# nevi-me/rust-dataframe

Hardware: AMD Instinct MI355X
Metric: rows/sec filter+sum over 1e9 f64 Arrow rows; %HBM bw at 1/2/4/8 GPU (higher is better)
Workload: dtype f64

## Files before the change

rust_dataframe_amd/csrc/rdf_capi.cpp:

```cpp
#include <hip/hip_runtime.h>

#include <algorithm>
#include <cmath>
#include <cstdarg>
#include <cstdio>
#include <chrono>
#include <functional>
#include <cstring>
#include <map>
#include <memory>
#include <mutex>
#include <condition_variable>
#include <string>
#include <thread>
#include <vector>
#include <sys/syscall.h>
#include <unistd.h>

#include "rdf_device.h"
#include "rdf_stage_copy.h"
#include "rdf_stream_plan.h"
#include "rdf_join_place.h"
#include "rdf_program_plan.h"
#include "rdf_groupby_multi_plan.h"
// ... 30 lines not shown
    std::vector<void*> overflow;
};

struct Ctx {
    bool        ready = false;
    int         device = 0;
    hipStream_t own_stream = nullptr;
    hipStream_t stream = nullptr;
    hipStream_t copy_stream = nullptr;
    bool copy_pending = false;
    Arena       arena;
    char*       pinned = nullptr;
    size_t      pinned_cap = 0;
    std::string err;
    std::string last_kernel;
    bool   opt_spec = true;
    bool   opt_fast_filter = true;
    bool   opt_vec_bitmap = false;
    int    opt_filter_block = 1;
    int    opt_interp_lean = 1;
    int    opt_filter_owned = 1;
    int    opt_filter_ends = 1;
    int    opt_filter_short = 1;
    int    opt_filter_block_rows = 8192;
    int    opt_filter_fused = 1;
    int    opt_gbm_route = 0;
    int64_t opt_gbm_slots = 0;
    int    opt_gb_debug = 0;
    bool   sort_used_local = false;
    int64_t utf8_sort_rounds = 0;
// ... 43 lines not shown
    char* tab_pin = nullptr; size_t tab_pin_cap = 0, tab_pin_used = 0;
    bool   agg_comm_entered = false;
    ::rdf_comm* agg_comm = nullptr;
    ~Ctx();
};

thread_local Ctx g_ctx;

Ctx::~Ctx() {
    if (!ready || (long)syscall(SYS_gettid) == (long)getpid()) return;
    (void)hipSetDevice(device);
    if (stream) (void)hipStreamSynchronize(stream);
    for (void* p : arena.overflow) (void)hipFree(p);
    if (arena.base) (void)hipFree(arena.base);
    if (pinned) (void)hipHostFree(pinned);
    for (auto& kv : pool_free) (void)hipFree(kv.second);
    for (int b = 0; b < 2; ++b) { if (sbuf_dev[b]) (void)hipFree(sbuf_dev[b]); if (sbuf_pin[b]) (void)hipHostFree(sbuf_pin[b]); if (sbuf_ev[b]) (void)hipEventDestroy(sbuf_ev[b]); }
    if (tab_pin) (void)hipHostFree(tab_pin);
    if (d2h_stream) (void)hipStreamSynchronize(d2h_stream);
    for (int b = 0; b < 2; ++b) { if (dbuf_dev[b]) (void)hipFree(dbuf_dev[b]); if (dbuf_pin[b]) (void)hipHostFree(dbuf_pin[b]); if (dbuf_ev[b]) (void)hipEventDestroy(dbuf_ev[b]); }
    if (d2h_stream) (void)hipStreamDestroy(d2h_stream);
    for (auto& ev : events) { (void)hipEventDestroy(ev.first); (void)hipEventDestroy(ev.second); }
    if (copy_stream) { (void)hipStreamSynchronize(copy_stream); (void)hipStreamDestroy(copy_stream); }
    if (own_stream) (void)hipStreamDestroy(own_stream);
    ready = false;
}

rdf_status fail(rdf_status st, const char* fmt, ...) {
    char buf[512];
    va_list ap;
// ... 19 lines not shown
rdf_status ensure_ready() {
    Ctx& c = g_ctx;
    if (c.ready) return RDF_OK;
    int n = 0;
    hipError_t e = hipGetDeviceCount(&n);
    if (e != hipSuccess || n <= 0)
        return fail(RDF_DEVICE_ERROR, "no HIP device visible (%s); librdf_mi355x has no CPU fallback",
                    e != hipSuccess ? hipGetErrorString(e) : "device count 0");
    HIP_TRY(hipGetDevice(&c.device));
    hipDeviceProp_t prop;
    HIP_TRY(hipGetDeviceProperties(&prop, c.device));
    if (strncmp(prop.gcnArchName, "gfx950", 6) != 0)
        return fail(RDF_DEVICE_ERROR, "device %d is %s; this library carries gfx950 (MI355X) code only", c.device, prop.gcnArchName);
    HIP_TRY(hipStreamCreateWithFlags(&c.own_stream, hipStreamNonBlocking));
    c.stream = c.own_stream;
    if (const char* e = getenv("RDF_SPEC_BLOCKS_PER_CU")) { const int v = atoi(e); if (v >= 0 && v <= 8) c.opt_spec_blocks = v; }
    if (const char* e = getenv("RDF_SPEC_TILE_ROT")) c.opt_spec_tile_rot = atoi(e);
    if (const char* e = getenv("RDF_SPEC_XCD_SWZ")) c.opt_spec_xcd_swz = atoi(e);
    if (const char* e = getenv("RDF_SPEC_GRID_ADJ")) c.opt_spec_grid_adj = atoi(e);
    if (const char* e = getenv("RDF_STREAM_TABLE_KERNEL")) c.opt_stream_table_kernel = atoi(e) != 0;
    if (const char* e = getenv("RDF_GSPEC_BLOCKS_PER_CU")) { const int v = atoi(e); if (v >= 0 && v <= 8) c.opt_gspec_blocks = v; }
    c.ready = true;
    return RDF_OK;
}

void arena_begin() {
    Arena& a = g_ctx.arena;
    for (void* p : a.overflow) (void)hipFree(p);
    a.overflow.clear();
    if (a.wanted > a.cap) {
// ... 138 lines not shown
        for (auto& it : items) if (!it.small) { it.off = off; off += (it.bytes + 16 + 255) & ~(size_t)255; }
        total = off;
        void* p = nullptr;
        RDF_TRY(arena_alloc(total ? total : 256, &p));
        dev = (char*)p;
        return RDF_OK;
    }
    char* ptr(int idx) const { return dev + items[(size_t)idx].off; }

    rdf_status upload(size_t pinned_off, size_t* pinned_used) {
        Ctx& c = g_ctx;
        if (small_bytes) {
            char* pin = c.pinned + pinned_off;
            packed_copy(items, pin, true, small_bytes);
            HIP_TRY(hipMemcpyAsync(dev, pin, small_bytes, hipMemcpyHostToDevice, c.stream));
        }
        *pinned_used = small_bytes;
        for (auto& it : items)
            if (!it.small && it.bytes) HIP_TRY(hipMemcpyAsync(dev + it.off, it.src, it.bytes, hipMemcpyHostToDevice, c.stream));
        return RDF_OK;
    }
    rdf_status download(size_t pinned_off) {
        Ctx& c = g_ctx;
        if (small_bytes) HIP_TRY(hipMemcpyAsync(c.pinned + pinned_off, dev, small_bytes, hipMemcpyDeviceToHost, c.stream));
        for (auto& it : items)
            if (!it.small && it.bytes) HIP_TRY(hipMemcpyAsync((void*)it.src, dev + it.off, it.bytes, hipMemcpyDeviceToHost, c.stream));
        HIP_TRY(hipStreamSynchronize(c.stream));
        if (small_bytes) {
            packed_copy(items, c.pinned + pinned_off, false, small_bytes);
        }
        return RDF_OK;
    }
};

struct InPlan {
    int values_item = -1, validity_item = -1;
    int64_t dev_offset = 0;
};

struct DbgTimer {
    bool on;
    std::chrono::steady_clock::time_point t0;
    DbgTimer() : on(getenv("RDF_DEBUG") != nullptr), t0(std::chrono::steady_clock::now()) {}
    void mark(const char* what) {
        if (!on) return;
        const auto t1 = std::chrono::steady_clock::now();
        fprintf(stderr, "[rdf] %-28s %8.3f ms\n", what, std::chrono::duration<double, std::milli>(t1 - t0).count());
        t0 = t1;
    }
};

struct InputStager {
    Region region;
    std::vector<InPlan> plans;
    std::vector<const rdf_array*> arrays;
    std::vector<DevChunkCol> dev;
    bool host = false;

    void add(const rdf_array* a) {
        arrays.push_back(a);
        if (a->mem != RDF_MEM_HOST && !host) return;
        if (plans.size() + 1 < arrays.size()) plans.resize(arrays.size() - 1);
// ... 56 lines not shown
        return RDF_OK;
    }
    template <typename T> T* at(size_t off) { return (T*)(base + off); }
    template <typename T> T* dev_at(size_t off) const { return (T*)(dev + off); }
    rdf_status alloc() {
        void* p = nullptr;
        RDF_TRY(arena_alloc(size ? size : 16, &p));
        dev = (char*)p;
        return RDF_OK;
    }
    rdf_status upload(size_t pinned_off) {
        Ctx& c = g_ctx;
        if (size == 0) return RDF_OK;
        if (base != c.pinned + pinned_off) return fail(RDF_COMPUTE_ERROR, "internal: table builder not bound to its staging offset");
        HIP_TRY(hipMemcpyAsync(dev, base, size, hipMemcpyHostToDevice, c.stream));
        return RDF_OK;
    }
};

rdf_status check_mem(const rdf_array* arrs, int64_t n, int32_t* mem_io) {
    for (int64_t i = 0; i < n; ++i) {
        if (arrs[i].mem != RDF_MEM_HOST && arrs[i].mem != RDF_MEM_DEVICE) return fail(RDF_INVALID_ARGUMENT, "bad mem tag %d", arrs[i].mem);
        if (*mem_io < 0) *mem_io = arrs[i].mem;
        else if (*mem_io != arrs[i].mem) return fail(RDF_INVALID_ARGUMENT, "all arrays of one call must share one memory space");
        if (arrs[i].length < 0 || arrs[i].offset < 0) return fail(RDF_INVALID_ARGUMENT, "negative length/offset");
        if (arrs[i].length > 0 && arrs[i].values == nullptr) return fail(RDF_INVALID_ARGUMENT, "null values pointer");
    }
    return RDF_OK;
}
rdf_status check_out_mem(const rdf_out* outs, int64_t n, int32_t mem) {
// ... 120 lines not shown
    hipError_t e = hipGetDeviceCount(&n);
    *count = e == hipSuccess ? n : 0;
    if (e != hipSuccess) return fail(RDF_DEVICE_ERROR, "hipGetDeviceCount: %s", hipGetErrorString(e));
    return RDF_OK;
}

rdf_status rdf_set_device(int32_t device) {
    Ctx& c = g_ctx;
    if (c.ready && c.device == device) return RDF_OK;
    if (c.ready) {
        (void)hipStreamSynchronize(c.stream);
        for (void* p : c.arena.overflow) (void)hipFree(p);
        c.arena.overflow.clear();
        if (c.arena.base) (void)hipFree(c.arena.base);
        c.arena = Arena();
        for (auto& ev : c.events) { (void)hipEventDestroy(ev.first); (void)hipEventDestroy(ev.second); }
        c.events.clear();
        c.events_used = 0;
        if (c.own_stream) (void)hipStreamDestroy(c.own_stream);
        c.own_stream = c.stream = nullptr;
        c.ready = false;
    }
    HIP_TRY(hipSetDevice(device));
    return ensure_ready();
}

rdf_status rdf_set_stream(void* hip_stream) {
    RDF_TRY(ensure_ready());
    g_ctx.stream = hip_stream ? (hipStream_t)hip_stream : g_ctx.own_stream;
    return RDF_OK;
// ... 1903 lines not shown
```

rust_dataframe_amd/csrc/rdf_capi_program.inc:

```

namespace {


bool op_is_arith(int op) { return op >= RDF_OP_ADD && op <= RDF_OP_DIV; }
bool op_is_fbinary(int op) { return op >= RDF_OP_ATAN2 && op <= RDF_OP_LOG; }
bool op_is_unary_math(int op) { return (op >= RDF_OP_ABS && op <= RDF_OP_TANH) || (op >= RDF_OP_COT && op <= RDF_OP_CSC); }
bool op_is_cmp(int op) { return op >= RDF_OP_GT && op <= RDF_OP_LE; }
bool op_is_hour(int op) { return op >= RDF_OP_HOUR_S && op <= RDF_OP_HOUR_DAY; }
bool op_is_binary(int op) { return op_is_arith(op) || op_is_fbinary(op) || op_is_cmp(op) || op == RDF_OP_AND || op == RDF_OP_OR; }
bool op_is_heavy(int op) {
    if (op_is_fbinary(op)) return true;
    if (!op_is_unary_math(op)) return false;
    switch (op) {
        case RDF_OP_ABS: case RDF_OP_CEIL: case RDF_OP_FLOOR: case RDF_OP_ROUND: case RDF_OP_SQRT:
        case RDF_OP_DEGREES: case RDF_OP_RADIANS: return false;
        default: return true;
    }
}

struct Compiler {
    const rdf_expr_node* nodes;
    int nnodes;
    const int* col_dtype;
    int ncols;
// ... 486 lines not shown
                    else if (op == RDF_OP_DIV) h = sw ? LH_F_RDIV : LH_F_DIV;
                } else if (in.dtype == RDF_I64 || in.dtype == RDF_U64) {
                    if (op == RDF_OP_ADD) h = LH_I_ADD;
                    else if (op == RDF_OP_MUL) h = LH_I_MUL;
                    else if (op == RDF_OP_SUB) h = sw ? LH_I_RSUB : LH_I_SUB;
                }
            } break;
            default: break;
        }
        if (h == LH_NONE) return false;
        lean.code[i].swapped = (uint8_t)((in.swapped & 1) | (h << 1));
    }
    return true;
}

rdf_status launch_agg_pair(const EvalArgs* ea, const FilterAggF64Args* fa, int cmp, int feat, int grid, int nvalues,
                           const int* cls, AggPartial* partials, AggPartial* result, const char* spec_sig = nullptr,
                           const SpecArgs* sa = nullptr) {
    Ctx& c = g_ctx;
    KernelTimer kt;
    if (sa) {
        const bool jit = jit_find(spec_sig) != nullptr;
        c.last_kernel = std::string("spec_kernel<") + spec_sig + ">" + (jit ? " [compiled at run time]" : "");
        const hipError_t le = launch_spec(spec_sig, *sa, grid, c.stream);
        if (le != hipSuccess && jit) { (void)hipGetLastError(); return kRetryInterpreted; }
        if (le != hipSuccess) return fail(RDF_DEVICE_ERROR, "launch_spec: %s", hipGetErrorString(le));
    }
    else if (fa) { c.last_kernel = "filter_agg_f64_kernel"; HIP_TRY(launch_filter_agg_f64(*fa, cmp, grid, c.stream)); }
    else {
        EvalArgs lean;
        if (c.opt_interp_lean && feat == 0 && lean_assign(*ea, lean)) { c.last_kernel = "eval_kernel<AGG, lean>"; HIP_TRY(launch_eval_lean(lean, SINK_AGG, grid, c.stream, c.opt_interp_lean == 2)); }
        else { c.last_kernel = "eval_kernel<AGG>"; HIP_TRY(launch_eval(*ea, SINK_AGG, feat, grid, c.stream)); }
    }
    kt.stop();
    AggFinalArgs f;
    memset(&f, 0, sizeof f);
    f.partials = partials;
    f.result = result;
    f.nblocks = grid;
    f.nvalues = nvalues;
    for (int k = 0; k < nvalues; ++k) f.value_cls[k] = cls[k];
    HIP_TRY(launch_agg_final(f, c.stream));
    return RDF_OK;
}

void fill_agg_result(rdf_agg_result* r, int dt, const AggPartial& p) {
    memset(r, 0, sizeof *r);
    r->dtype = dt;
    r->count = p.cnt;
    r->is_some = p.cnt > 0;
    if (is_float(dt)) {
        double s, a, b;
        memcpy(&s, &p.sum, 8); memcpy(&a, &p.mn, 8); memcpy(&b, &p.mx, 8);
        r->sum_f64 = dt == RDF_F32 ? (double)(float)s : s;
        if (p.cnt > 0) { r->min_f64 = a; r->max_f64 = b; }
    } else {
        r->sum_i64 = (int64_t)h_normalize_int(dt, p.sum);
        if (p.cnt > 0) { r->min_i64 = (int64_t)p.mn; r->max_i64 = (int64_t)p.mx; }
// ... 26 lines not shown
    int cls[kMaxGroupValues] = {0, 0, 0, 0, 0, 0, 0, 0};
    size_t pin_off = 0;
    InputStager in;
    const std::vector<DevChunkCol>* in_dev = nullptr;
    Region outr;
    std::vector<DevOutChunk> dev_outs;
    std::vector<int> out_val_item, out_vld_item;
    std::vector<int64_t> tile_start;
    const rdf_frame::Tiles* eval_tiles = nullptr;
    int64_t ntiles = 0;
    int grid = 0;
    size_t n_nc = 0;
    int gwords = 0;
    void* scratch = nullptr;
    uint32_t* d_flags = nullptr;
    int64_t* d_nullc = nullptr;
    AggPartial* d_partials = nullptr;
    AggPartial* d_result = nullptr;
    EvalArgs ea;
    TableBuilder tb;
    bool use_spec = false;
    SpecPlan sp;
    int rt_ops[8] = {0, 0, 0, 0, 0, 0, 0, 0};
    SpecArgs sa;
    TableBuilder stb;

    ProgramRun(const ProgramSpec& p, const rdf_array* c, int nc, int64_t nch, rdf_out* o, rdf_agg_result* a, rdf_frame* f)
        : ps(p), cols(c), ncols(nc), nchunks(nch), outs(o), aggs(a), fc(f), grouped(p.sink == RDF_SINK_GROUP), cc(p.nodes, p.nnodes, col_dtype, nc) {}
};

rdf_status program_check(ProgramRun& r, const char* len_mismatch_msg) {
    const ProgramSpec& ps = r.ps;
    const rdf_array* cols = r.cols;
    const int ncols = r.ncols;
    const int64_t nchunks = r.nchunks;
    rdf_frame* fc = r.fc;
    if (nchunks < 0) return fail(RDF_INVALID_ARGUMENT, "negative chunk count");
    if (ncols < 0 || ncols > kMaxCols) return fail(RDF_INVALID_ARGUMENT, "a fused program reads at most %d columns", kMaxCols);
    if (ps.nvalues < 1 || ps.nvalues > (r.grouped ? kMaxGroupValues : kMaxValues)) return fail(RDF_INVALID_ARGUMENT, "nvalues out of range");
    if (r.grouped) {
        if (ps.ngroups < 1 || (int64_t)(ps.ngroups + 1) * ps.nvalues > RDF_MAX_GROUP_SLOTS)
            return fail(RDF_INVALID_ARGUMENT, "grouped aggregation: (ngroups + 1) * nvalues must be in [2, %d] (large key domains: rdf_groupby_sum)", RDF_MAX_GROUP_SLOTS);
        if (!ps.gout) return fail(RDF_INVALID_ARGUMENT, "null output pointer");
// ... 91 lines not shown

rdf_status program_flags_status(uint32_t flags, const ProgramSpec& ps) {
    if ((flags & 2u) && ps.sink == RDF_SINK_AGG && g_ctx.agg_comm) return fail(RDF_COMPUTE_ERROR, "pipeline_dist: another rank failed before the combine");
    if (flags & 1u) return fail(RDF_DIVIDE_BY_ZERO, "Divide by zero error");
    if ((flags & 2u) && ps.sink == RDF_SINK_GROUP) return fail(RDF_COMPUTE_ERROR, "group id outside [0, %d)", ps.ngroups);
    return RDF_OK;
}

rdf_status deliver_agg(ProgramRun& r, const AggPartial* d_result, const uint32_t* d_flags) {
    Ctx& ctx = g_ctx;
    const int nvalues = r.ps.nvalues;
    AggPartial hp[kMaxValues];
    uint32_t flags = 0;
    if (ctx.agg_comm) RDF_TRY(agg_dist_finish(*ctx.agg_comm, d_result, d_flags, nvalues, r.cls, hp, &flags));
    else {
        RDF_TRY(pinned_reserve(r.pin_off + 64 + sizeof(AggPartial) * kMaxValues));
        char* pin = ctx.pinned + r.pin_off;
        HIP_TRY(hipMemcpyAsync(pin, d_flags, 16, hipMemcpyDeviceToHost, ctx.stream));
        HIP_TRY(hipMemcpyAsync(pin + 64, d_result, sizeof(AggPartial) * (size_t)nvalues, hipMemcpyDeviceToHost, ctx.stream));
        HIP_TRY(hipStreamSynchronize(ctx.stream));
        r.dbg.mark("kernel + result");
        memcpy(&flags, pin, 4);
        memcpy(hp, pin + 64, sizeof(AggPartial) * (size_t)nvalues);
    }
    RDF_TRY(program_flags_status(flags, r.ps));
    for (int v = 0; v < nvalues; ++v) fill_agg_result(&r.aggs[v], r.value_dtype[v], hp[v]);
    return RDF_OK;
}

rdf_status program_empty(ProgramRun& r) {
    const ProgramSpec& ps = r.ps;
    if (r.frame_store) return RDF_OK;
    if (ps.sink == RDF_SINK_STORE) {
        for (int64_t i = 0; i < (int64_t)ps.nvalues * r.nchunks; ++i) { r.outs[i].length = 0; r.outs[i].null_count = 0; }
    } else if (r.grouped) {
        for (int v = 0; v < ps.nvalues; ++v)
            for (int g = 0; g <= ps.ngroups; ++g) {
                rdf_group_result& gr = ps.gout[(size_t)v * (size_t)(ps.ngroups + 1) + (size_t)g];
                memset(&gr, 0, sizeof gr);
                gr.dtype = r.value_dtype[v];
// ... 23 lines not shown
    }
    return RDF_OK;
}

rdf_status program_stage(ProgramRun& r) {
    const ProgramSpec& ps = r.ps;
    const int64_t nchunks = r.nchunks;
    const int ncols = r.ncols;
    rdf_frame* fc = r.fc;
    RDF_TRY(ensure_ready());
    Ctx& ctx = g_ctx;
    arena_begin();
    size_t pin_used = 0;
    if (!fc) {
        r.in.arrays.reserve((size_t)ncols * (size_t)nchunks);
        r.in.plans.reserve((size_t)ncols * (size_t)nchunks);
        for (int64_t i = 0; i < (int64_t)ncols * nchunks; ++i) r.in.add(&r.cols[i]);
        RDF_TRY(r.in.finish(r.pin_off, &pin_used));
        r.pin_off += (pin_used + 255) & ~(size_t)255;
    }
    r.in_dev = fc ? &fc->dev : &r.in.dev;
    r.dbg.mark("stage inputs");

    const std::vector<int64_t>& clen = *r.clen;
    std::vector<DevOutChunk>& dev_outs = r.dev_outs;
    if (r.frame_store) {
        if (nchunks == 1) { dev_outs.resize((size_t)ps.nvalues); for (int v = 0; v < ps.nvalues; ++v) dev_outs[(size_t)v] = ps.frame_out0[v]; }
    } else if (ps.sink == RDF_SINK_STORE) {
        dev_outs.resize((size_t)ps.nvalues * nchunks);
        if (r.mem == RDF_MEM_HOST) {
            r.out_val_item.assign(dev_outs.size(), -1);
// ... 6 lines not shown
                    const size_t vb = r.value_dtype[v] == RDF_BOOL ? (size_t)((n + 7) / 8) : (size_t)n * (size_t)dtype_size(r.value_dtype[v]);
                    r.out_val_item[i] = r.outr.add(r.outs[i].values, vb);
                    if (r.outs[i].validity) r.out_vld_item[i] = r.outr.add(r.outs[i].validity, (size_t)((n + 7) / 8));
                }
            RDF_TRY(r.outr.layout());
            for (size_t i = 0; i < dev_outs.size(); ++i) {
                dev_outs[i].values = r.out_val_item[i] >= 0 ? r.outr.ptr(r.out_val_item[i]) : nullptr;
                dev_outs[i].validity = r.out_vld_item[i] >= 0 ? (uint8_t*)r.outr.ptr(r.out_vld_item[i]) : nullptr;
            }
        } else {
            for (size_t i = 0; i < dev_outs.size(); ++i) dev_outs[i] = DevOutChunk{r.outs[i].values, r.outs[i].validity};
        }
    }

    if (fc) { RDF_TRY(frame_tiles(*fc, kEvalTile, &r.eval_tiles)); r.ntiles = r.eval_tiles->ntiles; }
    else {
        r.tile_start.assign((size_t)nchunks + 1, 0);
        r.ntiles = tile_prefix(clen.data(), nchunks, kEvalTile, r.tile_start.data());
    }
    r.grid = (int)(r.ntiles < (int64_t)eval_grid_limit() ? r.ntiles : (int64_t)eval_grid_limit());

    r.n_nc = ps.sink == RDF_SINK_STORE ? (size_t)ps.nvalues * (size_t)nchunks : 0;
    r.gwords = r.grouped ? group_words(ps.ngroups, ps.nvalues) : 0;
    const size_t scratch_bytes = 16 + r.n_nc * 8 + ((size_t)r.grid + 4) * (r.grouped ? (size_t)r.gwords * 8 : (size_t)ps.nvalues * sizeof(AggPartial));
    RDF_TRY(arena_alloc(scratch_bytes, &r.scratch));
    r.d_flags = (uint32_t*)r.scratch;
    r.d_nullc = (int64_t*)((char*)r.scratch + 16);
    r.d_partials = (AggPartial*)((char*)r.scratch + 16 + r.n_nc * 8);
    r.d_result = r.d_partials + (size_t)r.grid * (size_t)ps.nvalues;
    HIP_TRY(hipMemsetAsync(r.scratch, 0, 16 + r.n_nc * 8, ctx.stream));

    EvalArgs& ea = r.ea;
    memset(&ea, 0, sizeof ea);
    ea.nchunks = nchunks;
    ea.ntiles = r.ntiles;
    ea.ncols = ncols;
    ea.nvalues = ps.nvalues;
    ea.ncode = (int)r.cc.code.size();
    ea.ntmp = r.cc.tmp_max;
    ea.flags = r.d_flags;
    ea.out_null_counts = r.d_nullc;
    ea.partials = r.d_partials;
    for (int k = 0; k < ncols; ++k) ea.col_dtype[k] = r.col_dtype[k];
    for (int v = 0; v < ps.nvalues; ++v) ea.value_cls[v] = r.cls[v];
    memcpy(ea.code, r.cc.code.data(), r.cc.code.size() * sizeof(Instr));
// ... 102 lines not shown
    for (int k = 0; k < kSpecCols; ++k) {
        sa.alias[k] = -1;
        for (int j = 0; j < k && k < sp.ncols; ++j) if (sp.col_map[j] == sp.col_map[k]) { sa.alias[k] = j; break; }
    }
    sa.partials = r.d_partials;
    sa.flags = r.d_flags;
    sa.vec_bitmap = ctx.opt_vec_bitmap ? 1 : 0;
    sa.out_null_count = r.d_nullc;
    sa.nchunks = nchunks;
    std::vector<int64_t> sts;
    const rdf_frame::Tiles* spec_tiles = nullptr;
    if (fc) {
        RDF_TRY(frame_tiles(*fc, spec_rpb, &spec_tiles));
        sa.ntiles = spec_tiles->ntiles;
        sa.tile_inv = spec_tiles->tile_inv;
    } else {
        sts.assign((size_t)nchunks + 1, 0);
        sa.ntiles = tile_prefix(clen.data(), nchunks, spec_rpb, sts.data());
        sa.tile_inv = tile_reciprocal(nchunks, sts[(size_t)nchunks - 1]);
    }
    if (nchunks == 1) {
        for (int k = 0; k < sp.ncols; ++k) sa.cols[k] = in_dev[(size_t)sp.col_map[k]];
        sa.n = clen[0];
        if (ps.sink == RDF_SINK_STORE) sa.out = r.dev_outs[0];
    } else if (fc) {
        DevChunkCol* tab = nullptr;
        RDF_TRY(frame_col_tab(*fc, sp.col_map, sp.ncols, &tab));
        sa.cols_tab = tab;
        sa.chunk_tile_start = spec_tiles->d_start;
        sa.chunk_len = fc->d_clen;
// ... 33 lines not shown
    wi.nchunks = nchunks;
    wi.ncols = sp.ncols;
    wi.any_bitmap = false;
    for (int k = 0; k < sp.ncols; ++k) wi.any_bitmap |= fc ? fc->col_nullable[sp.col_map[k]] : in_dev[(size_t)((int64_t)sp.col_map[k] * nchunks)].validity != nullptr;
    wi.ntiles = sa.ntiles;
    wi.grid_limit = eval_grid_limit();
    wi.waves_per_block = kBlock / 64;
    wi.spec_blocks_per_cu = ctx.opt_spec_blocks;
    wi.spec_tile_rot = ctx.opt_spec_tile_rot;
    wi.spec_xcd_swz = ctx.opt_spec_xcd_swz;
    wi.spec_grid_adj = ctx.opt_spec_grid_adj;
    const WalkPlan wp = spec_walk_plan(wi);
    r.grid = wp.grid;
    sa.tile_rot = wp.tile_rot;
    sa.xcd_swz = wp.xcd_swz;
    r.d_result = r.d_partials + (size_t)r.grid * (size_t)ps.nvalues;
    return RDF_OK;
}

rdf_status run_group(ProgramRun& r) {
    const ProgramSpec& ps = r.ps;
    Ctx& ctx = g_ctx;
    EvalArgs& ea = r.ea;
    const int64_t nchunks = r.nchunks;
    const std::vector<DevChunkCol>& in_dev = *r.in_dev;
    const std::vector<int64_t>& clen = *r.clen;
    const int gwords = r.gwords;
    ea.ngroups = ps.ngroups;
    ea.group_replicas = group_replicas(gwords, r.cc.tmp_max);
    uint64_t* d_gpart = (uint64_t*)r.d_partials;
    uint64_t* d_gres = d_gpart + (size_t)r.grid * (size_t)gwords;
    ea.group_partials = d_gpart;
    SpecPlan gp;
    bool use_gspec = ctx.opt_spec && ps.ngroups <= 8 &&
                     build_gspec_plan(r.cc, ps.filter_root, ps.group_root, ps.ngroups, ps.nvalues, ps.value_roots, gp);
    for (int k = 0; k < gp.ncols && use_gspec; ++k) {
        const int w = dtype_size(r.col_dtype[gp.col_map[k]]);
        for (int64_t c = 0; c < nchunks; ++c) {
            const DevChunkCol& d = in_dev[(size_t)((int64_t)gp.col_map[k] * nchunks + c)];
            if (clen[(size_t)c] > 0 && ((uintptr_t)((const char*)d.values + d.offset * w) & (uintptr_t)(2 * w - 1)) != 0) { use_gspec = false; break; }
        }
    }
    if (use_gspec) {
        GSpecArgs ga;
        memset(&ga, 0, sizeof ga);
        ga.cols_tab = ea.cols; ga.chunk_tile_start = ea.chunk_tile_start; ga.chunk_len = ea.chunk_len;
        ga.nchunks = nchunks; ga.ntiles = r.ntiles; ga.n = clen[0];
        for (int k = 0; k < gp.ncols; ++k) { ga.col_map[k] = gp.col_map[k]; if (nchunks == 1) ga.cols[k] = in_dev[(size_t)gp.col_map[k]]; }
        for (int k = 0; k < gp.nimm; ++k) ga.imm[k] = gp.imm[k];
        ga.group_partials = d_gpart; ga.flags = r.d_flags;
        ga.ngroups = ps.ngroups; ga.nvalues = ps.nvalues; ga.vec_bitmap = ctx.opt_vec_bitmap ? 1 : 0;
        const WalkPlan wp = gspec_walk_plan(r.grid, eval_grid_limit(), ctx.opt_gspec_blocks, ctx.opt_spec_tile_rot, ctx.opt_spec_xcd_swz);
        r.grid = wp.grid;
        ga.xcd_swz = wp.xcd_swz;
        ga.tile_rot = wp.tile_rot;
        KernelTimer kt;
        ctx.last_kernel = "gspec_kernel<" + gp.sig + ">" + (jit_find(gp.sig.c_str()) ? " [compiled at run time]" : "");
        const hipError_t le = launch_gspec(gp.sig.c_str(), ga, r.grid, ctx.stream);
        if (le != hipSuccess && jit_find(gp.sig.c_str()) == nullptr && !gspec_available(gp.sig.c_str())) {
            (void)hipGetLastError();
            return kRetryInterpreted;
        }
        if (le != hipSuccess) return fail(RDF_DEVICE_ERROR, "launch_gspec: %s", hipGetErrorString(le));
        kt.stop();
    } else {
        KernelTimer kt;
        ctx.last_kernel = "eval_kernel<GROUP>";
        HIP_TRY(launch_eval(ea, SINK_GROUP, r.cc.feat(), r.grid, ctx.stream));
        kt.stop();
    }
    GroupFinalArgs gf;
    memset(&gf, 0, sizeof gf);
    gf.partials = d_gpart; gf.result = d_gres; gf.nblocks = r.grid; gf.words = gwords; gf.ngroups = ps.ngroups; gf.nvalues = ps.nvalues;
    for (int v = 0; v < ps.nvalues; ++v) gf.value_cls[v] = r.cls[v];
    HIP_TRY(launch_group_final(gf, ctx.stream));
    RDF_TRY(pinned_reserve(r.pin_off + 64 + (size_t)gwords * 8));
    char* pin = ctx.pinned + r.pin_off;
    HIP_TRY(hipMemcpyAsync(pin, r.d_flags, 16, hipMemcpyDeviceToHost, ctx.stream));
    HIP_TRY(hipMemcpyAsync(pin + 64, d_gres, (size_t)gwords * 8, hipMemcpyDeviceToHost, ctx.stream));
    HIP_TRY(hipStreamSynchronize(ctx.stream));
    uint32_t flags;
    memcpy(&flags, pin, 4);
    RDF_TRY(program_flags_status(flags, ps));
    const uint64_t* w = (const uint64_t*)(pin + 64);
    const int S = ps.ngroups + 1;
    for (int v = 0; v < ps.nvalues; ++v)
        for (int g = 0; g < S; ++g) {
            rdf_group_result& gr = ps.gout[(size_t)v * (size_t)S + (size_t)g];
            memset(&gr, 0, sizeof gr);
            gr.dtype = r.value_dtype[v];
            gr.count = (int64_t)(w[2 * ps.nvalues * S + g] - w[(ps.nvalues + v) * S + g]);
            gr.is_some = gr.count > 0;
            if (is_float(r.value_dtype[v])) memcpy(&gr.sum_f64, &w[v * S + g], 8);
            else gr.sum_i64 = (int64_t)w[v * S + g];
        }
    if (ps.grows) for (int g = 0; g < S; ++g) ps.grows[g] = (int64_t)w[2 * ps.nvalues * S + g];
    return RDF_OK;
}

// ... 16 lines not shown
    if (!(coln && r.col_dtype[coln->column] == RDF_F64 && sc->dtype != RDF_NULLTYPE && (is_numeric(sc->dtype) || sc->dtype == RDF_BOOL))) return false;
    const DevChunkCol& x = (*r.in_dev)[(size_t)coln->column];
    const DevChunkCol& y = (*r.in_dev)[(size_t)vr.column];
    const uintptr_t xa = (uintptr_t)((const double*)x.values + x.offset), ya = (uintptr_t)((const double*)y.values + y.offset);
    if (!((xa & 7) == 0 && (ya & 7) == 0 && (xa & 15) == (ya & 15))) return false;
    memset(&fa, 0, sizeof fa);
    fa.x = (const double*)x.values; fa.x_validity = x.validity; fa.x_offset = x.offset;
    fa.y = (const double*)y.values; fa.y_validity = y.validity; fa.y_offset = y.offset;
    fa.n = (*r.clen)[0];
    const uint64_t cu = r.cc.imm_for(*sc, RDF_F64);
    memcpy(&fa.c, &cu, 8);
    fa.partials = r.d_partials;
    return true;
}

rdf_status run_agg(ProgramRun& r) {
    const ProgramSpec& ps = r.ps;
    FilterAggF64Args fa;
    int cmp = 0;
    if (r.use_spec) {
        RDF_TRY(launch_agg_pair(nullptr, nullptr, 0, 0, r.grid, ps.nvalues, r.cls, r.d_partials, r.d_result, r.sp.sig.c_str(), &r.sa));
    } else if (fast_filter_match(r, fa, cmp)) {
        const int64_t per_block = (int64_t)kBlock * 4 * 2;
        const int64_t want = ((*r.clen)[0] + per_block - 1) / per_block;
        r.grid = (int)(want < (int64_t)eval_grid_limit() ? want : (int64_t)eval_grid_limit());
        if (r.grid < 1) r.grid = 1;
        r.d_result = r.d_partials + (size_t)r.grid * (size_t)ps.nvalues;
        RDF_TRY(launch_agg_pair(nullptr, &fa, cmp, 0, r.grid, 1, r.cls, r.d_partials, r.d_result));
    } else {
        RDF_TRY(launch_agg_pair(&r.ea, nullptr, 0, r.cc.feat(), r.grid, ps.nvalues, r.cls, r.d_partials, r.d_result));
    }
    return deliver_agg(r, r.d_result, r.d_flags);
}

rdf_status run_store(ProgramRun& r) {
    const ProgramSpec& ps = r.ps;
    Ctx& ctx = g_ctx;
    const int64_t nchunks = r.nchunks;
    const std::vector<int64_t>& clen = *r.clen;
    {
        KernelTimer kt;
        if (r.use_spec) {
            const bool jit = jit_find(r.sp.sig.c_str()) != nullptr;
            ctx.last_kernel = "spec_kernel<" + r.sp.sig + ">" + (jit ? " [compiled at run time]" : "");
            const hipError_t le = launch_spec(r.sp.sig.c_str(), r.sa, r.grid, ctx.stream);
            if (le != hipSuccess && jit) { (void)hipGetLastError(); return kRetryInterpreted; }
            if (le != hipSuccess) return fail(RDF_DEVICE_ERROR, "launch_spec: %s", hipGetErrorString(le));
        }
        else {
            int64_t longest = 0;
            for (int64_t i = 0; i < nchunks; ++i) longest = std::max(longest, clen[(size_t)i]);
            EvalArgs lean;
            if (ctx.opt_interp_lean && r.cc.feat() == 0 && longest < ((int64_t)1 << 32) && lean_assign(r.ea, lean, SINK_STORE)) {
                ctx.last_kernel = "eval_kernel<STORE, lean>";
                HIP_TRY(launch_eval_lean(lean, SINK_STORE, r.grid, ctx.stream, ctx.opt_interp_lean == 2));
            } else { ctx.last_kernel = "eval_kernel<STORE>"; HIP_TRY(launch_eval(r.ea, SINK_STORE, r.cc.feat(), r.grid, ctx.stream)); }
        }
        kt.stop();
    }
    const size_t head = r.frame_store ? 16 : 16 + r.n_nc * 8;
    RDF_TRY(pinned_reserve(r.pin_off + 64 + (r.frame_store ? 0 : r.n_nc * 8 + r.outr.small_bytes + 256)));
    char* pin = ctx.pinned + r.pin_off;
    HIP_TRY(hipMemcpyAsync(pin, r.scratch, head, hipMemcpyDeviceToHost, ctx.stream));
    if (!r.frame_store && r.mem == RDF_MEM_HOST) RDF_TRY(r.outr.download(r.pin_off + ((head + 255) & ~(size_t)255)));
    else HIP_TRY(hipStreamSynchronize(ctx.stream));
    uint32_t flags;
    memcpy(&flags, pin, 4);
    RDF_TRY(program_flags_status(flags, ps));
    if (r.frame_store) return RDF_OK;
    for (int v = 0; v < ps.nvalues; ++v)
        for (int64_t c = 0; c < nchunks; ++c) {
            rdf_out& o = r.outs[(int64_t)v * nchunks + c];
            o.length = clen[(size_t)c];
            memcpy(&o.null_count, pin + 16 + 8 * (size_t)((int64_t)v * nchunks + c), 8);
        }
    return RDF_OK;
}

// ... 87 lines not shown
```

rust_dataframe_amd/csrc/rdf_device.h:

```cpp
#pragma once
#include "rdf_sort_map.h"
#include <stdint.h>
#include <hip/hip_runtime.h>

#include <string>
#include "../../include/rdf_mi355x.h"

namespace rdfk {

constexpr int kBlock = 256;
constexpr int kVPT = 4;
constexpr int kEvalTile = kBlock * kVPT;
constexpr int kFilterTile = 4096;
constexpr int kMaxCode = 56;
constexpr int kMaxCols = 8;
constexpr int kMaxFrameCols = 64;
constexpr int kPreCols = 4;
constexpr int kMaxTmp = 4;
constexpr int kMaxValues = RDF_MAX_VALUES;
constexpr int kMaxGroupValues = RDF_MAX_GROUP_VALUES;
constexpr int kMaxFilterCols = 8;

struct DevChunkCol {
    const void*    values;
// ... 59 lines not shown
constexpr int kGSpecImm = 8;
struct GSpecArgs {
    const DevChunkCol* cols_tab;
    const int64_t*     chunk_tile_start;
    const int64_t*     chunk_len;
    DevChunkCol        cols[kGSpecCols];
    int32_t            col_map[kGSpecCols];
    int64_t            nchunks, ntiles, n;
    uint64_t           imm[kGSpecImm];
    uint64_t*          group_partials;
    uint32_t*          flags;
    int32_t            ngroups, nvalues, vec_bitmap;
    int32_t            xcd_swz, tile_rot, pad1;
};

struct GroupFinalArgs {
    const uint64_t* partials;
    uint64_t*       result;
    int32_t         nblocks, words, ngroups, nvalues;
    int32_t         value_cls[kMaxGroupValues];
};

struct AggFinalArgs {
    const AggPartial* partials;
    AggPartial*       result;
    int32_t           nblocks, nvalues;
    int32_t           value_cls[kMaxValues];
};

struct FilterAggF64Args {
    const double*  x;   const uint8_t* x_validity;   int64_t x_offset;
    const double*  y;   const uint8_t* y_validity;   int64_t y_offset;
    int64_t        n;
    double         c;
    AggPartial*    partials;
};

constexpr int kSpecCols = 8;
constexpr int kSpecImm = 8;
struct SpecArgs {
    DevChunkCol        cols[kSpecCols];
    DevOutChunk        out;
// ... 602 lines not shown
```

rust_dataframe_amd/csrc/rdf_kernels.hip:

```cpp
#include "rdf_common.hip.h"

namespace rdfk {

__global__ __launch_bounds__(kBlock) void agg_final_kernel(const AggFinalArgs a) {
    __shared__ AggPartial red_lds[kBlock / 64];
    for (int k = 0; k < a.nvalues; ++k) {
        const int cls = a.value_cls[k];
        uint64_t s, mn, mx;
        int64_t cnt;
        agg_init(cls, s, mn, mx, cnt);
        for (int b = threadIdx.x; b < a.nblocks; b += kBlock) {
            const AggPartial p = a.partials[(int64_t)b * a.nvalues + k];
            agg_merge(cls, s, mn, mx, cnt, p.sum, p.mn, p.mx, p.cnt);
        }
        block_reduce_agg(cls, s, mn, mx, cnt, red_lds, &a.result[k]);
        __syncthreads();
    }
}


template <int CMP>
__device__ __forceinline__ bool cmp_f64(double x, double c) {
    if (CMP == RDF_OP_GT) return x > c;
    if (CMP == RDF_OP_GE) return x >= c;
// ... 775 lines not shown
    return limit;
}

hipError_t launch_eval_feat0(const EvalArgs& a, int sink, int grid, hipStream_t s);
hipError_t launch_eval_feat1(const EvalArgs& a, int sink, int grid, hipStream_t s);
hipError_t launch_eval_feat2(const EvalArgs& a, int sink, int grid, hipStream_t s);
hipError_t launch_eval(const EvalArgs& a, int sink, int feat, int grid, hipStream_t s) {
    if (feat <= 0) return launch_eval_feat0(a, sink, grid, s);
    if (feat == 1) return launch_eval_feat1(a, sink, grid, s);
    return launch_eval_feat2(a, sink, grid, s);
}

__global__ __launch_bounds__(64) void group_final_kernel(const GroupFinalArgs a) {
    const int w = blockIdx.x, lane = threadIdx.x;
    const int S = a.ngroups + 1;
    const bool fsum = w < a.nvalues * S && a.value_cls[(w / S) & (kMaxGroupValues - 1)] == CLS_F64;
    uint64_t acc = 0;
    if (fsum) {
        double d = 0.0;
        for (int b = lane; b < a.nblocks; b += 64) d += u2d(a.partials[(size_t)b * a.words + w]);
        acc = d2u(d);
    } else {
        for (int b = lane; b < a.nblocks; b += 64) acc += a.partials[(size_t)b * a.words + w];
    }
#pragma unroll
    for (int m = 32; m >= 1; m >>= 1) {
        const uint64_t y = shfl_xor64(acc, m);
        acc = fsum ? d2u(u2d(acc) + u2d(y)) : acc + y;
    }
    if (lane == 0) a.result[w] = acc;
// ... 163 lines not shown
```

Measured before the change: 851.7 billion.

## Reuse persistent device flags and merge result readback into one copy

Agg and group paths now use a persistent per-context flags word that the final reduction kernel copies into a header right before the result and then clears. This removes the per-call memset unless a previous call left the flags dirty, and merges the two D2H copies into one. Spec kernel name strings are cached, and single-chunk inputs skip the tile-start vector allocation. The gain is a few microseconds of launch overhead per call, which is small against a 1e9-row scan. If a call errors before the flags are cleared, it relies on the dirty bit to stay correct.

```diff
diff --git a/rust_dataframe_amd/csrc/rdf_capi.cpp b/rust_dataframe_amd/csrc/rdf_capi.cpp
--- a/rust_dataframe_amd/csrc/rdf_capi.cpp
+++ b/rust_dataframe_amd/csrc/rdf_capi.cpp
@@ -68,6 +68,12 @@
     size_t      pinned_cap = 0;
     std::string err;
     std::string last_kernel;
+    std::string named_sig, named_kernel;
+    const char* named_base = nullptr;
+    bool   named_jit = false;
+    uint32_t* d_call_flags = nullptr;
+    bool   call_flags_dirty = true;
+    int    ops_memset = 0, ops_kernel = 0, ops_copy = 0;
     bool   opt_spec = true;
     bool   opt_fast_filter = true;
     bool   opt_vec_bitmap = false;
@@ -141,6 +147,7 @@
     for (void* p : arena.overflow) (void)hipFree(p);
     if (arena.base) (void)hipFree(arena.base);
     if (pinned) (void)hipHostFree(pinned);
+    if (d_call_flags) (void)hipFree(d_call_flags);
     for (auto& kv : pool_free) (void)hipFree(kv.second);
     for (int b = 0; b < 2; ++b) { if (sbuf_dev[b]) (void)hipFree(sbuf_dev[b]); if (sbuf_pin[b]) (void)hipHostFree(sbuf_pin[b]); if (sbuf_ev[b]) (void)hipEventDestroy(sbuf_ev[b]); }
     if (tab_pin) (void)hipHostFree(tab_pin);
@@ -190,6 +197,8 @@
         return fail(RDF_DEVICE_ERROR, "device %d is %s; this library carries gfx950 (MI355X) code only", c.device, prop.gcnArchName);
     HIP_TRY(hipStreamCreateWithFlags(&c.own_stream, hipStreamNonBlocking));
     c.stream = c.own_stream;
+    HIP_TRY(hipMalloc((void**)&c.d_call_flags, 256));
+    c.call_flags_dirty = true;
     if (const char* e = getenv("RDF_SPEC_BLOCKS_PER_CU")) { const int v = atoi(e); if (v >= 0 && v <= 8) c.opt_spec_blocks = v; }
     if (const char* e = getenv("RDF_SPEC_TILE_ROT")) c.opt_spec_tile_rot = atoi(e);
     if (const char* e = getenv("RDF_SPEC_XCD_SWZ")) c.opt_spec_xcd_swz = atoi(e);
@@ -358,17 +367,18 @@
             char* pin = c.pinned + pinned_off;
             packed_copy(items, pin, true, small_bytes);
             HIP_TRY(hipMemcpyAsync(dev, pin, small_bytes, hipMemcpyHostToDevice, c.stream));
+            ++c.ops_copy;
         }
         *pinned_used = small_bytes;
         for (auto& it : items)
-            if (!it.small && it.bytes) HIP_TRY(hipMemcpyAsync(dev + it.off, it.src, it.bytes, hipMemcpyHostToDevice, c.stream));
+            if (!it.small && it.bytes) { HIP_TRY(hipMemcpyAsync(dev + it.off, it.src, it.bytes, hipMemcpyHostToDevice, c.stream)); ++c.ops_copy; }
         return RDF_OK;
     }
     rdf_status download(size_t pinned_off) {
         Ctx& c = g_ctx;
-        if (small_bytes) HIP_TRY(hipMemcpyAsync(c.pinned + pinned_off, dev, small_bytes, hipMemcpyDeviceToHost, c.stream));
+        if (small_bytes) { HIP_TRY(hipMemcpyAsync(c.pinned + pinned_off, dev, small_bytes, hipMemcpyDeviceToHost, c.stream)); ++c.ops_copy; }
         for (auto& it : items)
-            if (!it.small && it.bytes) HIP_TRY(hipMemcpyAsync((void*)it.src, dev + it.off, it.bytes, hipMemcpyDeviceToHost, c.stream));
+            if (!it.small && it.bytes) { HIP_TRY(hipMemcpyAsync((void*)it.src, dev + it.off, it.bytes, hipMemcpyDeviceToHost, c.stream)); ++c.ops_copy; }
         HIP_TRY(hipStreamSynchronize(c.stream));
         if (small_bytes) {
             packed_copy(items, c.pinned + pinned_off, false, small_bytes);
@@ -389,7 +399,7 @@
     void mark(const char* what) {
         if (!on) return;
         const auto t1 = std::chrono::steady_clock::now();
-        fprintf(stderr, "[rdf] %-28s %8.3f ms\n", what, std::chrono::duration<double, std::milli>(t1 - t0).count());
+        fprintf(stderr, "[rdf] %-28s %9.4f ms\n", what, std::chrono::duration<double, std::milli>(t1 - t0).count());
         t0 = t1;
     }
 };
@@ -476,6 +486,7 @@
         if (size == 0) return RDF_OK;
         if (base != c.pinned + pinned_off) return fail(RDF_COMPUTE_ERROR, "internal: table builder not bound to its staging offset");
         HIP_TRY(hipMemcpyAsync(dev, base, size, hipMemcpyHostToDevice, c.stream));
+        ++c.ops_copy;
         return RDF_OK;
     }
 };
@@ -626,6 +637,8 @@
         c.arena.overflow.clear();
         if (c.arena.base) (void)hipFree(c.arena.base);
         c.arena = Arena();
+        if (c.d_call_flags) (void)hipFree(c.d_call_flags);
+        c.d_call_flags = nullptr;
         for (auto& ev : c.events) { (void)hipEventDestroy(ev.first); (void)hipEventDestroy(ev.second); }
         c.events.clear();
         c.events_used = 0;
diff --git a/rust_dataframe_amd/csrc/rdf_capi_program.inc b/rust_dataframe_amd/csrc/rdf_capi_program.inc
--- a/rust_dataframe_amd/csrc/rdf_capi_program.inc
+++ b/rust_dataframe_amd/csrc/rdf_capi_program.inc
@@ -524,34 +524,14 @@
     return true;
 }
 
-rdf_status launch_agg_pair(const EvalArgs* ea, const FilterAggF64Args* fa, int cmp, int feat, int grid, int nvalues,
-                           const int* cls, AggPartial* partials, AggPartial* result, const char* spec_sig = nullptr,
-                           const SpecArgs* sa = nullptr) {
-    Ctx& c = g_ctx;
-    KernelTimer kt;
-    if (sa) {
-        const bool jit = jit_find(spec_sig) != nullptr;
-        c.last_kernel = std::string("spec_kernel<") + spec_sig + ">" + (jit ? " [compiled at run time]" : "");
-        const hipError_t le = launch_spec(spec_sig, *sa, grid, c.stream);
-        if (le != hipSuccess && jit) { (void)hipGetLastError(); return kRetryInterpreted; }
-        if (le != hipSuccess) return fail(RDF_DEVICE_ERROR, "launch_spec: %s", hipGetErrorString(le));
-    }
-    else if (fa) { c.last_kernel = "filter_agg_f64_kernel"; HIP_TRY(launch_filter_agg_f64(*fa, cmp, grid, c.stream)); }
-    else {
-        EvalArgs lean;
-        if (c.opt_interp_lean && feat == 0 && lean_assign(*ea, lean)) { c.last_kernel = "eval_kernel<AGG, lean>"; HIP_TRY(launch_eval_lean(lean, SINK_AGG, grid, c.stream, c.opt_interp_lean == 2)); }
-        else { c.last_kernel = "eval_kernel<AGG>"; HIP_TRY(launch_eval(*ea, SINK_AGG, feat, grid, c.stream)); }
-    }
-    kt.stop();
-    AggFinalArgs f;
-    memset(&f, 0, sizeof f);
-    f.partials = partials;
-    f.result = result;
-    f.nblocks = grid;
-    f.nvalues = nvalues;
-    for (int k = 0; k < nvalues; ++k) f.value_cls[k] = cls[k];
-    HIP_TRY(launch_agg_final(f, c.stream));
-    return RDF_OK;
+void name_spec_kernel(Ctx& c, const char* kernel, const std::string& sig, bool jit) {
+    if (c.named_jit != jit || c.named_sig != sig || !c.named_base || strcmp(c.named_base, kernel) != 0) {
+        c.named_base = kernel;
+        c.named_jit = jit;
+        c.named_sig = sig;
+        c.named_kernel = std::string(kernel) + "<" + sig + ">" + (jit ? " [compiled at run time]" : "");
+    }
+    if (c.last_kernel != c.named_kernel) c.last_kernel = c.named_kernel;
 }
 
 void fill_agg_result(rdf_agg_result* r, int dt, const AggPartial& p) {
@@ -608,9 +588,12 @@
     int gwords = 0;
     void* scratch = nullptr;
     uint32_t* d_flags = nullptr;
+    bool own_flags = false;
     int64_t* d_nullc = nullptr;
     AggPartial* d_partials = nullptr;
     AggPartial* d_result = nullptr;
+    char* result_header() const { return (char*)d_partials + (size_t)grid * (grouped ? (size_t)gwords * 8 : (size_t)ps.nvalues * sizeof(AggPartial)); }
+    void place_result() { d_result = (AggPartial*)(result_header() + kResultHeaderBytes); }
     EvalArgs ea;
     TableBuilder tb;
     bool use_spec = false;
@@ -620,7 +603,10 @@
     TableBuilder stb;
 
     ProgramRun(const ProgramSpec& p, const rdf_array* c, int nc, int64_t nch, rdf_out* o, rdf_agg_result* a, rdf_frame* f)
-        : ps(p), cols(c), ncols(nc), nchunks(nch), outs(o), aggs(a), fc(f), grouped(p.sink == RDF_SINK_GROUP), cc(p.nodes, p.nnodes, col_dtype, nc) {}
+        : ps(p), cols(c), ncols(nc), nchunks(nch), outs(o), aggs(a), fc(f), grouped(p.sink == RDF_SINK_GROUP), cc(p.nodes, p.nnodes, col_dtype, nc) {
+        g_ctx.ops_memset = g_ctx.ops_kernel = g_ctx.ops_copy = 0;
+    }
+    ~ProgramRun() { if (dbg.on) fprintf(stderr, "[rdf] stream operations: %d memsets, %d kernels, %d copies\n", g_ctx.ops_memset, g_ctx.ops_kernel, g_ctx.ops_copy); }
 };
 
 rdf_status program_check(ProgramRun& r, const char* len_mismatch_msg) {
@@ -742,16 +728,18 @@
     uint32_t flags = 0;
     if (ctx.agg_comm) RDF_TRY(agg_dist_finish(*ctx.agg_comm, d_result, d_flags, nvalues, r.cls, hp, &flags));
     else {
-        RDF_TRY(pinned_reserve(r.pin_off + 64 + sizeof(AggPartial) * kMaxValues));
+        static_assert(kResultHeaderBytes == 64, "the pinned image of the result block: header, then the values");
+        RDF_TRY(pinned_reserve(r.pin_off + kResultHeaderBytes + sizeof(AggPartial) * kMaxValues));
         char* pin = ctx.pinned + r.pin_off;
-        HIP_TRY(hipMemcpyAsync(pin, d_flags, 16, hipMemcpyDeviceToHost, ctx.stream));
-        HIP_TRY(hipMemcpyAsync(pin + 64, d_result, sizeof(AggPartial) * (size_t)nvalues, hipMemcpyDeviceToHost, ctx.stream));
+        HIP_TRY(hipMemcpyAsync(pin, (const char*)d_result - kResultHeaderBytes, kResultHeaderBytes + sizeof(AggPartial) * (size_t)nvalues, hipMemcpyDeviceToHost, ctx.stream));
+        ++ctx.ops_copy;
         HIP_TRY(hipStreamSynchronize(ctx.stream));
         r.dbg.mark("kernel + result");
         memcpy(&flags, pin, 4);
-        memcpy(hp, pin + 64, sizeof(AggPartial) * (size_t)nvalues);
+        memcpy(hp, pin + kResultHeaderBytes, sizeof(AggPartial) * (size_t)nvalues);
     }
     RDF_TRY(program_flags_status(flags, r.ps));
+    if (r.own_flags) ctx.call_flags_dirty = false;
     for (int v = 0; v < nvalues; ++v) fill_agg_result(&r.aggs[v], r.value_dtype[v], hp[v]);
     return RDF_OK;
 }
@@ -805,7 +793,7 @@
     size_t pin_used = 0;
     if (!fc) {
         r.in.arrays.reserve((size_t)ncols * (size_t)nchunks);
-        r.in.plans.reserve((size_t)ncols * (size_t)nchunks);
+        if (r.mem == RDF_MEM_HOST) r.in.plans.reserve((size_t)ncols * (size_t)nchunks);
         for (int64_t i = 0; i < (int64_t)ncols * nchunks; ++i) r.in.add(&r.cols[i]);
         RDF_TRY(r.in.finish(r.pin_off, &pin_used));
         r.pin_off += (pin_used + 255) & ~(size_t)255;
@@ -842,7 +830,10 @@
     }
 
     if (fc) { RDF_TRY(frame_tiles(*fc, kEvalTile, &r.eval_tiles)); r.ntiles = r.eval_tiles->ntiles; }
-    else {
+    else if (nchunks == 1) {
+        int64_t ts[2] = {0, 0};
+        r.ntiles = tile_prefix(clen.data(), 1, kEvalTile, ts);
+    } else {
         r.tile_start.assign((size_t)nchunks + 1, 0);
         r.ntiles = tile_prefix(clen.data(), nchunks, kEvalTile, r.tile_start.data());
     }
@@ -850,13 +841,21 @@
 
     r.n_nc = ps.sink == RDF_SINK_STORE ? (size_t)ps.nvalues * (size_t)nchunks : 0;
     r.gwords = r.grouped ? group_words(ps.ngroups, ps.nvalues) : 0;
-    const size_t scratch_bytes = 16 + r.n_nc * 8 + ((size_t)r.grid + 4) * (r.grouped ? (size_t)r.gwords * 8 : (size_t)ps.nvalues * sizeof(AggPartial));
+    const size_t scratch_bytes = 16 + r.n_nc * 8 + kResultHeaderBytes + ((size_t)r.grid + 4) * (r.grouped ? (size_t)r.gwords * 8 : (size_t)ps.nvalues * sizeof(AggPartial));
     RDF_TRY(arena_alloc(scratch_bytes, &r.scratch));
     r.d_flags = (uint32_t*)r.scratch;
     r.d_nullc = (int64_t*)((char*)r.scratch + 16);
     r.d_partials = (AggPartial*)((char*)r.scratch + 16 + r.n_nc * 8);
-    r.d_result = r.d_partials + (size_t)r.grid * (size_t)ps.nvalues;
-    HIP_TRY(hipMemsetAsync(r.scratch, 0, 16 + r.n_nc * 8, ctx.stream));
+    r.place_result();
+    r.own_flags = r.grouped || (ps.sink == RDF_SINK_AGG && !ctx.agg_comm);
+    if (r.own_flags) {
+        r.d_flags = ctx.d_call_flags;
+        if (ctx.call_flags_dirty) { HIP_TRY(hipMemsetAsync(r.d_flags, 0, 16, ctx.stream)); ++ctx.ops_memset; }
+        ctx.call_flags_dirty = true;
+    } else {
+        HIP_TRY(hipMemsetAsync(r.scratch, 0, 16 + r.n_nc * 8, ctx.stream));
+        ++ctx.ops_memset;
+    }
 
     EvalArgs& ea = r.ea;
     memset(&ea, 0, sizeof ea);
@@ -989,6 +988,10 @@
         RDF_TRY(frame_tiles(*fc, spec_rpb, &spec_tiles));
         sa.ntiles = spec_tiles->ntiles;
         sa.tile_inv = spec_tiles->tile_inv;
+    } else if (nchunks == 1) {
+        int64_t ts[2] = {0, 0};
+        sa.ntiles = tile_prefix(clen.data(), 1, spec_rpb, ts);
+        sa.tile_inv = tile_reciprocal(1, ts[0]);
     } else {
         sts.assign((size_t)nchunks + 1, 0);
         sa.ntiles = tile_prefix(clen.data(), nchunks, spec_rpb, sts.data());
@@ -1052,7 +1055,7 @@
     r.grid = wp.grid;
     sa.tile_rot = wp.tile_rot;
     sa.xcd_swz = wp.xcd_swz;
-    r.d_result = r.d_partials + (size_t)r.grid * (size_t)ps.nvalues;
+    r.place_result();
     return RDF_OK;
 }
 
@@ -1067,7 +1070,6 @@
     ea.ngroups = ps.ngroups;
     ea.group_replicas = group_replicas(gwords, r.cc.tmp_max);
     uint64_t* d_gpart = (uint64_t*)r.d_partials;
-    uint64_t* d_gres = d_gpart + (size_t)r.grid * (size_t)gwords;
     ea.group_partials = d_gpart;
     SpecPlan gp;
     bool use_gspec = ctx.opt_spec && ps.ngroups <= 8 &&
@@ -1093,7 +1095,7 @@
         ga.xcd_swz = wp.xcd_swz;
         ga.tile_rot = wp.tile_rot;
         KernelTimer kt;
-        ctx.last_kernel = "gspec_kernel<" + gp.sig + ">" + (jit_find(gp.sig.c_str()) ? " [compiled at run time]" : "");
+        name_spec_kernel(ctx, "gspec_kernel", gp.sig, jit_find(gp.sig.c_str()) != nullptr);
         const hipError_t le = launch_gspec(gp.sig.c_str(), ga, r.grid, ctx.stream);
         if (le != hipSuccess && jit_find(gp.sig.c_str()) == nullptr && !gspec_available(gp.sig.c_str())) {
             (void)hipGetLastError();
@@ -1109,18 +1111,24 @@
     }
     GroupFinalArgs gf;
     memset(&gf, 0, sizeof gf);
+    r.place_result();
+    uint64_t* d_gres = (uint64_t*)r.d_result;
     gf.partials = d_gpart; gf.result = d_gres; gf.nblocks = r.grid; gf.words = gwords; gf.ngroups = ps.ngroups; gf.nvalues = ps.nvalues;
     for (int v = 0; v < ps.nvalues; ++v) gf.value_cls[v] = r.cls[v];
+    gf.flags = r.d_flags; gf.header = (uint32_t*)r.result_header();
     HIP_TRY(launch_group_final(gf, ctx.stream));
-    RDF_TRY(pinned_reserve(r.pin_off + 64 + (size_t)gwords * 8));
+    ctx.ops_kernel += 2;
+    RDF_TRY(pinned_reserve(r.pin_off + kResultHeaderBytes + (size_t)gwords * 8));
     char* pin = ctx.pinned + r.pin_off;
-    HIP_TRY(hipMemcpyAsync(pin, r.d_flags, 16, hipMemcpyDeviceToHost, ctx.stream));
-    HIP_TRY(hipMemcpyAsync(pin + 64, d_gres, (size_t)gwords * 8, hipMemcpyDeviceToHost, ctx.stream));
+    HIP_TRY(hipMemcpyAsync(pin, r.result_header(), kResultHeaderBytes + (size_t)gwords * 8, hipMemcpyDeviceToHost, ctx.stream));
+    ++ctx.ops_copy;
     HIP_TRY(hipStreamSynchronize(ctx.stream));
+    r.dbg.mark("kernel + result");
     uint32_t flags;
     memcpy(&flags, pin, 4);
     RDF_TRY(program_flags_status(flags, ps));
-    const uint64_t* w = (const uint64_t*)(pin + 64);
+    ctx.call_flags_dirty = false;
+    const uint64_t* w = (const uint64_t*)(pin + kResultHeaderBytes);
     const int S = ps.ngroups + 1;
     for (int v = 0; v < ps.nvalues; ++v)
         for (int g = 0; g < S; ++g) {
@@ -1167,21 +1175,52 @@
     return true;
 }
 
+rdf_status launch_agg_pair(ProgramRun& r, const EvalArgs* ea, const FilterAggF64Args* fa, int cmp, int feat, const SpecArgs* sa = nullptr) {
+    Ctx& c = g_ctx;
+    const int grid = r.grid, nvalues = r.ps.nvalues;
+    KernelTimer kt;
+    if (sa) {
+        const char* spec_sig = r.sp.sig.c_str();
+        const bool jit = jit_find(spec_sig) != nullptr;
+        name_spec_kernel(c, "spec_kernel", r.sp.sig, jit);
+        const hipError_t le = launch_spec(spec_sig, *sa, grid, c.stream);
+        if (le != hipSuccess && jit) { (void)hipGetLastError(); return kRetryInterpreted; }
+        if (le != hipSuccess) return fail(RDF_DEVICE_ERROR, "launch_spec: %s", hipGetErrorString(le));
+    }
+    else if (fa) { c.last_kernel = "filter_agg_f64_kernel"; HIP_TRY(launch_filter_agg_f64(*fa, cmp, grid, c.stream)); }
+    else {
+        EvalArgs lean;
+        if (c.opt_interp_lean && feat == 0 && lean_assign(*ea, lean)) { c.last_kernel = "eval_kernel<AGG, lean>"; HIP_TRY(launch_eval_lean(lean, SINK_AGG, grid, c.stream, c.opt_interp_lean == 2)); }
+        else { c.last_kernel = "eval_kernel<AGG>"; HIP_TRY(launch_eval(*ea, SINK_AGG, feat, grid, c.stream)); }
+    }
+    kt.stop();
+    AggFinalArgs f;
+    memset(&f, 0, sizeof f);
+    f.partials = r.d_partials;
+    f.result = r.d_result;
+    f.nblocks = grid;
+    f.nvalues = nvalues;
+    for (int k = 0; k < nvalues; ++k) f.value_cls[k] = r.cls[k];
+    if (r.own_flags) { f.flags = r.d_flags; f.header = (uint32_t*)r.result_header(); }
+    HIP_TRY(launch_agg_final(f, c.stream));
+    c.ops_kernel += 2;
+    return RDF_OK;
+}
+
 rdf_status run_agg(ProgramRun& r) {
-    const ProgramSpec& ps = r.ps;
     FilterAggF64Args fa;
     int cmp = 0;
     if (r.use_spec) {
-        RDF_TRY(launch_agg_pair(nullptr, nullptr, 0, 0, r.grid, ps.nvalues, r.cls, r.d_partials, r.d_result, r.sp.sig.c_str(), &r.sa));
+        RDF_TRY(launch_agg_pair(r, nullptr, nullptr, 0, 0, &r.sa));
     } else if (fast_filter_match(r, fa, cmp)) {
         const int64_t per_block = (int64_t)kBlock * 4 * 2;
         const int64_t want = ((*r.clen)[0] + per_block - 1) / per_block;
         r.grid = (int)(want < (int64_t)eval_grid_limit() ? want : (int64_t)eval_grid_limit());
         if (r.grid < 1) r.grid = 1;
-        r.d_result = r.d_partials + (size_t)r.grid * (size_t)ps.nvalues;
-        RDF_TRY(launch_agg_pair(nullptr, &fa, cmp, 0, r.grid, 1, r.cls, r.d_partials, r.d_result));
+        r.place_result();
+        RDF_TRY(launch_agg_pair(r, nullptr, &fa, cmp, 0));
     } else {
-        RDF_TRY(launch_agg_pair(&r.ea, nullptr, 0, r.cc.feat(), r.grid, ps.nvalues, r.cls, r.d_partials, r.d_result));
+        RDF_TRY(launch_agg_pair(r, &r.ea, nullptr, 0, r.cc.feat()));
     }
     return deliver_agg(r, r.d_result, r.d_flags);
 }
@@ -1195,7 +1234,7 @@
         KernelTimer kt;
         if (r.use_spec) {
             const bool jit = jit_find(r.sp.sig.c_str()) != nullptr;
-            ctx.last_kernel = "spec_kernel<" + r.sp.sig + ">" + (jit ? " [compiled at run time]" : "");
+            name_spec_kernel(ctx, "spec_kernel", r.sp.sig, jit);
             const hipError_t le = launch_spec(r.sp.sig.c_str(), r.sa, r.grid, ctx.stream);
             if (le != hipSuccess && jit) { (void)hipGetLastError(); return kRetryInterpreted; }
             if (le != hipSuccess) return fail(RDF_DEVICE_ERROR, "launch_spec: %s", hipGetErrorString(le));
@@ -1210,11 +1249,13 @@
             } else { ctx.last_kernel = "eval_kernel<STORE>"; HIP_TRY(launch_eval(r.ea, SINK_STORE, r.cc.feat(), r.grid, ctx.stream)); }
         }
         kt.stop();
+        ++ctx.ops_kernel;
     }
     const size_t head = r.frame_store ? 16 : 16 + r.n_nc * 8;
     RDF_TRY(pinned_reserve(r.pin_off + 64 + (r.frame_store ? 0 : r.n_nc * 8 + r.outr.small_bytes + 256)));
     char* pin = ctx.pinned + r.pin_off;
     HIP_TRY(hipMemcpyAsync(pin, r.scratch, head, hipMemcpyDeviceToHost, ctx.stream));
+    ++ctx.ops_copy;
     if (!r.frame_store && r.mem == RDF_MEM_HOST) RDF_TRY(r.outr.download(r.pin_off + ((head + 255) & ~(size_t)255)));
     else HIP_TRY(hipStreamSynchronize(ctx.stream));
     uint32_t flags;
diff --git a/rust_dataframe_amd/csrc/rdf_device.h b/rust_dataframe_amd/csrc/rdf_device.h
--- a/rust_dataframe_amd/csrc/rdf_device.h
+++ b/rust_dataframe_amd/csrc/rdf_device.h
@@ -97,11 +97,15 @@
     int32_t            xcd_swz, tile_rot, pad1;
 };
 
+constexpr int kResultHeaderBytes = 64;
+
 struct GroupFinalArgs {
     const uint64_t* partials;
     uint64_t*       result;
     int32_t         nblocks, words, ngroups, nvalues;
     int32_t         value_cls[kMaxGroupValues];
+    uint32_t*       flags;
+    uint32_t*       header;
 };
 
 struct AggFinalArgs {
@@ -109,6 +113,8 @@
     AggPartial*       result;
     int32_t           nblocks, nvalues;
     int32_t           value_cls[kMaxValues];
+    uint32_t*         flags;
+    uint32_t*         header;
 };
 
 struct FilterAggF64Args {
diff --git a/rust_dataframe_amd/csrc/rdf_kernels.hip b/rust_dataframe_amd/csrc/rdf_kernels.hip
--- a/rust_dataframe_amd/csrc/rdf_kernels.hip
+++ b/rust_dataframe_amd/csrc/rdf_kernels.hip
@@ -1,9 +1,16 @@
 #include "rdf_common.hip.h"
 
 namespace rdfk {
+
+__device__ __forceinline__ void deliver_flags(uint32_t* flags, uint32_t* header) {
+    if (!flags || !header) return;
+    *header = *flags;
+    *flags = 0;
+}
 
 __global__ __launch_bounds__(kBlock) void agg_final_kernel(const AggFinalArgs a) {
     __shared__ AggPartial red_lds[kBlock / 64];
+    if (threadIdx.x == 0) deliver_flags(a.flags, a.header);
     for (int k = 0; k < a.nvalues; ++k) {
         const int cls = a.value_cls[k];
         uint64_t s, mn, mx;
@@ -813,6 +820,7 @@
 __global__ __launch_bounds__(64) void group_final_kernel(const GroupFinalArgs a) {
     const int w = blockIdx.x, lane = threadIdx.x;
     const int S = a.ngroups + 1;
+    if (w == 0 && lane == 0) deliver_flags(a.flags, a.header);
     const bool fsum = w < a.nvalues * S && a.value_cls[(w / S) & (kMaxGroupValues - 1)] == CLS_F64;
     uint64_t acc = 0;
     if (fsum) {
```

Measured after the change: 850.8 billion. Within noise of the previous version (-0.1%).
